# istellartech/GELATO

Measured on AMD Instinct MI355X. Metric: residual+Jacobian evals/sec (and ms/eval), 6-phase x 64-node LGR mesh, higher is better.
Workload: dtype f64

## Files before the change

### gelato_amd/csrc/gel_device.h

```cpp
#pragma once
#include <hip/hip_runtime.h>
#include <stdint.h>

namespace gel {

struct PhaseDev {
  int32_t n, ua, xa;
  int32_t air;
  int32_t air_fd;
  int32_t t_fd;
  int32_t q_fd;
  int32_t engine_on;
  int32_t hold;
  int32_t K;
  int32_t s_vv, s_vq, s_vt, s_qq;
  int32_t doff;
  int32_t toff;
  int64_t voff;
  double thrust, massflow, area, nozzle;
  double mf_um;
};

#ifdef __HIPCC__
template <class T>
__device__ __forceinline__ T load_const(const T* p) {
  return *(const T __attribute__((address_space(4)))*)p;
}
__device__ __forceinline__ int4 load_const_int4(const int4* p) {
  const int32_t* ip = (const int32_t*)p;
  int4 v;
  v.x = load_const(ip); v.y = load_const(ip + 1); v.z = load_const(ip + 2); v.w = load_const(ip + 3);
  return v;
}
__device__ __forceinline__ PhaseDev load_phase(const PhaseDev* g) {
  PhaseDev q;
  q.n = load_const(&g->n); q.ua = load_const(&g->ua); q.xa = load_const(&g->xa);
  q.air = load_const(&g->air); q.air_fd = load_const(&g->air_fd); q.t_fd = load_const(&g->t_fd); q.q_fd = load_const(&g->q_fd); q.engine_on = load_const(&g->engine_on);
  q.hold = load_const(&g->hold); q.K = load_const(&g->K);
  q.s_vv = load_const(&g->s_vv); q.s_vq = load_const(&g->s_vq); q.s_vt = load_const(&g->s_vt); q.s_qq = load_const(&g->s_qq);
  q.doff = load_const(&g->doff); q.toff = load_const(&g->toff); q.voff = load_const(&g->voff);
  q.thrust = load_const(&g->thrust); q.massflow = load_const(&g->massflow); q.area = load_const(&g->area);
  q.nozzle = load_const(&g->nozzle); q.mf_um = load_const(&g->mf_um);
  return q;
}
#endif

// ... 68 lines not shown
```

### gelato_amd/csrc/gel_eval_kernel.h

```cpp
#pragma once

namespace gel {

enum ParkSlot { PK_Q0 = 0, PK_Q1, PK_Q2, PK_Q3, PK_V0, PK_V1, PK_V2, PK_DJJ, PK_LV0, PK_LV1, PK_LV2,
                PK_FP0, PK_FP1, PK_FP2, PK_FP3, PK_FP4, PK_FP5, PK_FP6, PK_FP7, PK_COUNT };
constexpr int kStageLd = 17;
constexpr int kWaveLds = PK_COUNT * 64;
static_assert(kWaveLds >= 64 * kStageLd, "the MFMA staging tile must fit the wave's park region");
constexpr int kCoopStageOff = PK_LV0 * 64;
static_assert(kWaveLds - kCoopStageOff >= 64 * 11, "the cooperative hand-over area must fit behind the early park slots");
constexpr int kXldsPipeFrom = kLongPhaseFrom;
constexpr int kSlabRowsMax = 68, kPackRows = 36, kParkRes = (PK_LV2 + 1) * 64;
constexpr int kPipeSlabK = 8;
constexpr int wave_lds_doubles(bool jac, bool mfma, bool pack, bool split = false, bool longp = true) {
  return jac ? kWaveLds : (!mfma ? kParkRes : (split ? 64 * kStageLd  : (pack ? kParkRes + 4 * 64  : (longp ? 2 * 4 * kPipeSlabK * 11 + 64 * kPipeSlabK  : kSlabRowsMax * 11))));
}
static_assert(wave_lds_doubles(false, true, false, true) >= kParkRes, "residual-only split form: park over the result tile");
static_assert(wave_lds_doubles(false, true, true) >= 64 * 11 && wave_lds_doubles(false, true, false) >= 64 * 11 && wave_lds_doubles(false, true, false, false, false) >= 64 * 11, "hand-over area");
static_assert(wave_lds_doubles(false, true, true) >= kParkRes && wave_lds_doubles(false, true, false) >= kParkRes && wave_lds_doubles(false, true, false, false, false) >= kParkRes, "residual-only park");

constexpr int kSlotPT = 0, kSlotVM = 3, kSlotVP = 6;

#ifndef GEL_MIN_WAVES_PER_SIMD
#define GEL_MIN_WAVES_PER_SIMD 4
#endif
#ifndef GEL_MIN_WAVES_PER_SIMD_PACKJAC
#define GEL_MIN_WAVES_PER_SIMD_PACKJAC 4
#endif
#ifndef GEL_MIN_WAVES_PER_SIMD_RES
#define GEL_MIN_WAVES_PER_SIMD_RES 5
#endif

typedef double gel_double4 __attribute__((ext_vector_type(4)));

#ifndef GEL_CA_CACHE
#define GEL_CA_CACHE 1
#endif
#ifndef GEL_XLDS_A_PF_JAC
#define GEL_XLDS_A_PF_JAC 4
#endif
#ifndef GEL_XLDS_A_PF_RES
#define GEL_XLDS_A_PF_RES 4
#endif
#ifndef GEL_PACK_A_PRELOAD
#define GEL_PACK_A_PRELOAD 1
#endif


// ... 102 lines not shown
  const int dsw = __builtin_amdgcn_readfirstlane(ck.z);
  const int j = PACK ? (lane & 31) : j0 + lane;
  const PhaseDev ph = load_phase((COOP ? f_phases : P.phases) + sec);
  const bool csplit = SPLIT && MFMA && !JAC && B == 1 && res != nullptr && P.split_vel && !((P.unit0 | P.nunits) & 3);
  const bool only_dx = SPLIT && part && (!ph.air || !JAC);
  if (only_dx && !csplit) return;
  const bool lead = !(SPLIT && part);
  const int n = ph.n;
  const bool active = j < n;
  if (!MFMA && !active) return;
  const int jc = active ? j : n - 1;
  const int g = ph.ua + j;
  const int xj = ph.xa + 1 + jc;
  const int M = P.M, N = P.N;

  const double* xb = x + (size_t)b * P.nvars;
  const double* xm = xb;
  const double* xr = xb + M;
  const double* xv = xb + 4 * M;
  const double* xq = xb + 7 * M;
  const double* xu = xb + 11 * M;
  const double* xt = xb + 11 * M + 2 * N;
#define GEL_UNI(v) (PACK ? (v) : wave_uniform(v))
#ifndef GEL_KNOT_VLOAD
#define GEL_KNOT_VLOAD 1
#endif
  int sec_ld = sec;
  if (GEL_KNOT_VLOAD && JAC && !SPLIT) asm volatile("" : "+v"(sec_ld));
  const double to_ld = xt[sec_ld], tf_ld = xt[sec_ld + 1];
  double to = 0.0, tf = 0.0, fds = 0.0, fdt = 0.0;
  const double dx = P.dx, ut = P.ut;
  const double hT = P.hT;
  const double inv_dx = P.inv_dx;
#define GEL_TAKE_KNOT_TIMES()                                   \
  do {                                                          \
    to = GEL_UNI(to_ld); tf = GEL_UNI(tf_ld);                   \
    fds = GEL_UNI(inv_dx * (tf - to) * ut / 2.0);               \
    fdt = GEL_UNI(inv_dx * ut / 2.0);                           \
  } while (0)
  unsigned long long bad = 0;
#define GEL_CHK(v) (bad |= __builtin_amdgcn_ballot_w64(!(fabs(v) <= 1.79769313486231570815e308)))
  const bool packed = SPLIT && P.shard_width != 0;
  const int nn = min(64, n - j0);
  const int sub_hi = packed ? (part ? kSlotVP + 3 * (part - 1) : (ph.air ? 9 : 0)) : 0;
// ... 86 lines not shown
        if (twin_) d_[(W) * (n + lane) + c_] = -(vals_)[c_];                                                           \
      }                                                                                                                \
    }                                                                                                                  \
  } while (0)
#define EMIT_GROUP(W, slot0, vals_, g, k, twin_, okl_)                                                                 \
  do {                                                                                                                 \
    if (coo) {                                                                                                         \
      GEL_COO_EMIT(W, GEL_COO_BASE(g) + (size_t)(W) * n * (k), vals_, okl_, twin_);                                    \
    } else if (okl_) {                                                                                                 \
      _Pragma("unroll") for (int c_ = 0; c_ < (W); c_++) EMIT((slot0) + c_, (vals_)[c_]);                              \
    }                                                                                                                  \
  } while (0)

  constexpr bool XLDS = COOP;
  double me = 0.0, re[3] = {0.0, 0.0, 0.0};
  if (!XLDS) { me = xm[xj]; re[0] = xr[3 * xj]; re[1] = xr[3 * xj + 1]; re[2] = xr[3 * xj + 2]; }
  const double tau = P.tau[ph.toff + jc];
  {
    double q[4] = {0.0, 0.0, 0.0, 0.0}, ve[3] = {0.0, 0.0, 0.0};
    if (!XLDS) {
#pragma unroll
      for (int c = 0; c < 4; c++) q[c] = xq[4 * xj + c];
#pragma unroll
      for (int c = 0; c < 3; c++) ve[c] = xv[3 * xj + c];
    }
    double u0 = 0.0, u1 = 0.0;
    if (!ph.hold) { u0 = xu[2 * (ph.ua + jc)]; u1 = xu[2 * (ph.ua + jc) + 1]; }
    const double djj = JAC ? P.Dt[ph.doff + (size_t)(jc + 1) * n + jc] : 0.0;
    const bool tail1 = MFMA && ((n + 1) & 3) == 1 && n >= 4;
    const int ksteps = tail1 ? (n >> 2) : ((n + 4) >> 2);
    const double* const dcol = P.Dt + ph.doff + (size_t)n * n;
    double dl4[4] = {0, 0, 0, 0};
    if (COOP && tail1) {
      const int rt = PACK ? (wv & 1) : wv;
#pragma unroll
      for (int i = 0; i < 4; i++) dl4[i] = dcol[min(j0 + 16 * rt + (lane >> 4) + 4 * i, n - 1)];
    }
    const double dlast = (SPLIT && tail1) ? dcol[jc] : 0.0;
    double xl[11] = {0, 0, 0, 0, 0, 0, 0, 0, 0, 0, 0};
#define GEL_DX_TAIL_ACC(nct_, xn_of_ct)                                                             \
  do {                                                                                              \
    if (tail1) {                                                                                    \
      _Pragma("unroll") for (int ct = 0; ct < 3; ct++) {                                            \
        if (ct < (nct_)) {                                   \
          const double xn_ = (xn_of_ct);                                                            \
          _Pragma("unroll") for (int i = 0; i < 4; i++) acc[ct][i] = __builtin_fma(dl4[i], xn_, acc[ct][i]); \
        }                                                                                           \
      }                                                                                             \
    }                                                                                               \
  } while (0)

    double m0 = 0.0, q0[4] = {0, 0, 0, 0};
    bool ref0_done = false;
// ... 6 lines not shown
        static_assert(!COOP || kSlabRows * 11 <= kWL, "a slab of state rows must fit the wave's park region");
        lds_double* regions = (lds_double*)lds + park_off;
        const bool h7 = GEL_DX_HOLD7 && !PACK && ph.hold;
        const int ncv = h7 ? 7 : 11;
        const int ncols = ncv * kVecWg;
        const int ct0 = PACK ? (h7 ? 2 : 3) * (wv >> 1) : 0;
        int xoff[3];
#pragma unroll
        for (int ct = 0; ct < 3; ct++) {
          const int c = 16 * (ct0 + ct) + c16;
          const int vb = min(h7 ? c / 7 : c / 11, kVecWg - 1);
          const int col = (c < ncols) ? c - ncv * vb : 0;
          xoff[ct] = PACK ? (vb >> 1) * kWL + (vb & 1) * kPackRows * 11 + col + kq * 11 : vb * kWL + col + kq * 11;
        }
        gel_double4 acc[3];
        const double* ap = P.Dst + (size_t)dsw * 4 + (PACK ? (wv & 1) : wv) * 64 + lane;
        constexpr int kAPF = JAC ? GEL_XLDS_A_PF_JAC : GEL_XLDS_A_PF_RES;
        constexpr int kAllN = PACK ? 9 : kSlabK;
        constexpr bool kAAll = PACK ? (GEL_PACK_A_PRELOAD != 0) : (kAPF >= kSlabK);
        double a_all[kAAll ? kAllN : 1], a_ring[kAAll ? 1 : kAPF];
        if (kAAll) {
#pragma unroll
          for (int ks = 0; ks < kAllN; ks++) a_all[ks] = ap[min(ks, ksteps - 1) * 256];
        } else {
#pragma unroll
          for (int i = 0; i < kAPF; i++) a_ring[i] = ap[min(i, ksteps - 1) * 256];
        }
        constexpr int kRowsStaged = PACK ? 2 * kPackRows : kSlabRows, kExtra = (kRowsStaged - 64) * 11;
        double st[11], sx[(kExtra + 63) / 64];
        {
          const int hv = PACK ? lane / kPackRows : 0;
          const int k = PACK ? lane - kPackRows * hv : lane;
          const double* xs = PACK ? x + (size_t)min(b0 + 2 * wv + hv, B - 1) * P.nvars : xb;
          const int xk = ph.xa + min(k, n);
          st[0] = xs[xk];
#pragma unroll
          for (int c = 0; c < 3; c++) { st[1 + c] = xs[M + 3 * xk + c]; st[4 + c] = xs[4 * M + 3 * xk + c]; }
#pragma unroll
          for (int c = 0; c < 4; c++) st[7 + c] = xs[7 * M + 4 * xk + c];
          constexpr int kER = kRowsStaged - 64, kERs = (kER == 8) ? 3 : 2;
          static_assert(kER == (1 << kERs) && (!PACK || 64 >= kPackRows), "extra rows: a power of two, all in the second half");
#pragma unroll
          for (int i = 0; i < (kExtra + 63) / 64; i++) {
            const int e = min(lane + 64 * i, kExtra - 1);
            const int rr = 64 + (e & (kER - 1)), c = e >> kERs;
            const int kx = min(PACK ? rr - kPackRows : rr, n);
            const double* xe = PACK ? x + (size_t)min(b0 + 2 * wv + 1, B - 1) * P.nvars : xb;
            const int xr_ = ph.xa + kx;
            const int off = (c == 0) ? xr_ : ((c < 4) ? M + 3 * xr_ + (c - 1) : ((c < 7) ? 4 * M + 3 * xr_ + (c - 4) : 7 * M + 4 * xr_ + (c - 7)));
            sx[i] = xe[off];
          }
          lds_double* dst = wave_lds + lane * 11;
#pragma unroll
          for (int c = 0; c < 11; c++) dst[c] = st[c];
#pragma unroll
          for (int i = 0; i < (kExtra + 63) / 64; i++) {
            const int e = min(lane + 64 * i, kExtra - 1);
            wave_lds[(64 + (e & (kER - 1))) * 11 + (e >> kERs)] = sx[i];
          }
        }
        stage_tables_commit(P, lds, tab_mine);
        __syncthreads();
        const int klast = ksteps;
#define GEL_DX_ONE_SLAB(kTiles)                                                                                          \
  do {                                                                                                                   \
// ... 9 lines not shown
            acc[ct] = __builtin_amdgcn_mfma_f64_16x16x4f64(a_all[ks], bl_[ct], ks ? acc[ct] : zero4, 0, 0, 0);           \
        }                                                                                                                \
      }                                                                                                                  \
    } else {                                                                                                             \
       \
      _Pragma("unroll") for (int ct = 0; ct < 3; ct++) acc[ct] = gel_double4{0.0, 0.0, 0.0, 0.0};                        \
      for (int ks = 0; ks < klast; ks += kAPF) {                                                                         \
        _Pragma("unroll") for (int i = 0; i < kAPF; i++) {                                                               \
          if (ks + i < klast) {                                                                        \
            const int ro = (ks + i) * 44;                                                                                \
            double bl_[kTiles];                                                                                          \
            _Pragma("unroll") for (int ct = 0; ct < (kTiles); ct++) bl_[ct] = regions[xoff[ct] + ro];                    \
            _Pragma("unroll") for (int ct = 0; ct < (kTiles); ct++)                                                      \
              acc[ct] = __builtin_amdgcn_mfma_f64_16x16x4f64(a_ring[i], bl_[ct], acc[ct], 0, 0, 0);                      \
          }                                                                                                              \
          a_ring[i] = ap[min(ks + i + kAPF, ksteps - 1) * 256];                                                          \
        }                                                                                                                \
      }                                                                                                                  \
    }                                                                                                                    \
  } while (0)
        if (h7) GEL_DX_ONE_SLAB(2); else GEL_DX_ONE_SLAB(3);
#undef GEL_DX_ONE_SLAB
        GEL_DX_TAIL_ACC(h7 ? 2 : 3, regions[xoff[ct] + (n - kq) * 11]);
        {
          lds_double* src = wave_lds + (half * kPackRows + jc + 1) * 11;
          me = src[0];
#pragma unroll
          for (int c = 0; c < 3; c++) { re[c] = src[1 + c]; ve[c] = src[4 + c]; }
#pragma unroll
          for (int c = 0; c < 4; c++) q[c] = src[7 + c];
          lds_double* src0 = wave_lds + (half * kPackRows) * 11;
          if (!ph.engine_on) m0 = src0[0];
          if (ph.hold) {
#pragma unroll
            for (int c = 0; c < 4; c++) q0[c] = src0[7 + c];
          }
          ref0_done = true;
// ... 43 lines not shown
          xstr[ct] = stride;
        }
        gel_double4 acc[3];
#pragma unroll
        for (int ct = 0; ct < 3; ct++) acc[ct] = gel_double4{0.0, 0.0, 0.0, 0.0};
        typedef const __attribute__((address_space(1))) void* gel_gptr;
        typedef __attribute__((address_space(3))) void* gel_lptr;
        const int xa0 = ph.xa;
        const int s0 = (lane < 16) ? xa0 + 2 * lane : M + 3 * xa0 + 2 * (lane - 16);
        const int s1 = (lane < 48) ? 4 * M + 3 * xa0 + 2 * lane : 7 * M + 4 * xa0 + 2 * (lane - 48);
        const int s2 = 7 * M + 4 * xa0 + 2 * (16 + lane);
        const int a0 = (lane < 16) ? kPipeRows : 3 * kPipeRows, a1 = (lane < 48) ? 3 * kPipeRows : 4 * kPipeRows, a2 = 4 * kPipeRows;
#define GEL_PIPE_ROWS(slab, buf)                                                                                   \
  do {                                                                                                             \
    lds_double* _img = wave_lds + (buf) * kPipeBuf;                                                                \
    __builtin_amdgcn_global_load_lds((gel_gptr)(xb + s0 + (slab) * a0), (gel_lptr)_img, 16, 0, 0);                 \
    __builtin_amdgcn_global_load_lds((gel_gptr)(xb + s1 + (slab) * a1), (gel_lptr)(_img + 128), 16, 0, 0);         \
    if (lane < 48) __builtin_amdgcn_global_load_lds((gel_gptr)(xb + s2 + (slab) * a2), (gel_lptr)(_img + 256), 16, 0, 0); \
  } while (0)
        const double* ap2 = P.Dst + (size_t)dsw * 4 + wv * 64 + (lane & 31) * 2;
        const int khalf = lane >> 5, kmax = ((n + 4) >> 2) - 1;
#define GEL_PIPE_A(pair, k)                                                                                        \
  __builtin_amdgcn_global_load_lds((gel_gptr)(ap2 + (size_t)min((k) + khalf, kmax) * 256), (gel_lptr)(wave_lds + kRingOff + 128 * (pair)), 16, 0, 0)
#define GEL_PIPE_WAIT(N) asm volatile("s_waitcnt vmcnt(%0)" ::"n"(N) : "memory")
        GEL_PIPE_ROWS(0, 0);
#pragma unroll
        for (int pr = 0; pr < kPairs; pr++) GEL_PIPE_A(pr, 2 * pr);
        stage_tables_commit(P, lds, tab_mine);
        GEL_PIPE_WAIT(0);
        __syncthreads();
        const int nslab = (((n + 4) >> 2) + kPipeK - 1) / kPipeK;
        const int own = jc + 1;
        const lds_double* ring = wave_lds + kRingOff + lane;
        for (int sl = 0; sl < nslab; sl++) {
          const int bo = (sl & 1) * kPipeBuf;
          const bool more = sl + 1 < nslab;
          const int k0 = sl * kPipeK;
          if (more) GEL_PIPE_ROWS(sl + 1, (sl + 1) & 1);
// ... 63 lines not shown
          if (c < ncols && (ct < 2 || !h7)) {
#pragma unroll
            for (int i = 0; i < 4; i++) wg_lds[vb * kWL + (16 * wv + kq + 4 * i) * 11 + col] = acc[ct][i];
          }
        }
        __syncthreads();
        if (ghost) return;
        lds_double* row = wave_lds + kHO + lane * 11;
        lm = row[0];
#pragma unroll
        for (int c = 0; c < 3; c++) { lr[c] = row[1 + c]; lv[c] = row[4 + c]; }
#pragma unroll
        for (int c = 0; c < 4; c++) lq[c] = row[7 + c];
      } else if (MFMA && csplit) {
        const int c16 = lane & 15, kq = lane >> 4;
        const double* bp = xm + ph.xa;
        int bs = 1;
        if (c16 >= 1 && c16 < 4) { bp = xr + 3 * ph.xa + (c16 - 1); bs = 3; }
        if (c16 >= 4 && c16 < 7) { bp = xv + 3 * ph.xa + (c16 - 4); bs = 3; }
        if (c16 >= 7) { bp = xq + 4 * ph.xa + ((c16 < 11) ? (c16 - 7) : 0); bs = 4; }
        gel_double4 acc1 = gel_double4{0.0, 0.0, 0.0, 0.0};
        const double* ap1 = P.Dst + (size_t)dsw * 4 + part * 64 + lane;
        const unsigned un = (unsigned)n, ubs = (unsigned)bs;
        if (tail1 && rb) {
          xl[0] = xm[ph.xa + n];
#pragma unroll
          for (int c = 0; c < 3; c++) { xl[1 + c] = xr[3 * (ph.xa + n) + c]; xl[4 + c] = xv[3 * (ph.xa + n) + c]; }
#pragma unroll
          for (int c = 0; c < 4; c++) xl[7 + c] = xq[4 * (ph.xa + n) + c];
        }
        constexpr int kSplitB = SPLITB, kSplitA = 4;
        if (n < kSlabRowsMax) {
          static_assert(!(SPLIT && MFMA && !JAC) || kSlabRowsMax * 11 <= kWL, "the state-row image must fit a wavefront's region");
          lds_double* img = wave_lds + (1 - part) * kWL;
          constexpr int kQRows = kSlabRowsMax / 4, kQ = kQRows * 11;
#pragma unroll
          for (int i = 0; i < (kQ + 63) / 64; i++) {
            const int e = lane + 64 * i;
            const int rl = (e * 373) >> 12, c = e - 11 * rl;
            const int r = kQRows * part + rl;
            if (e < kQ) {
              const int xr_ = ph.xa + min(r, n);
              const int off = (c == 0) ? xr_ : ((c < 4) ? M + 3 * xr_ + (c - 1) : ((c < 7) ? 4 * M + 3 * xr_ + (c - 4) : 7 * M + 4 * xr_ + (c - 7)));
              const double v = xb[off];
              img[r * 11 + c] = (r <= n) ? v : 0.0;
            }
          }
          double a1[kSplitA];
#pragma unroll
          for (int i = 0; i < kSplitA; i++) a1[i] = ap1[min(i, ksteps - 1) * 256];
          __syncthreads();
          const int bo = kq * 11 + ((c16 < 11) ? c16 : 0);
#pragma unroll
          for (int i = 0; i < kSlabRowsMax / 4; i++) {
            if (i < ksteps) {
              acc1 = __builtin_amdgcn_mfma_f64_16x16x4f64(a1[i % kSplitA], img[bo + 44 * i], acc1, 0, 0, 0);
              a1[i % kSplitA] = ap1[min(i + kSplitA, ksteps - 1) * 256];
            }
          }
        } else {
          for (int k0 = 0; k0 < ksteps; k0 += kSplitB) {
            double bl[kSplitB], a1[kSplitA];
#pragma unroll
            for (int i = 0; i < kSplitB; i++) bl[i] = bp[min(4u * (k0 + i) + kq, un) * ubs];
#pragma unroll
            for (int i = 0; i < kSplitA; i++) a1[i] = ap1[min(k0 + i, ksteps - 1) * 256];
#pragma unroll
            for (int i = 0; i < kSplitB; i++) {
              if (k0 + i < ksteps) {
                acc1 = __builtin_amdgcn_mfma_f64_16x16x4f64(a1[i % kSplitA], bl[i], acc1, 0, 0, 0);
                a1[i % kSplitA] = ap1[min(k0 + i + kSplitA, ksteps - 1) * 256];
              }
            }
          }
        }
        lds_double* lead_lds = wave_lds - part * kWL;
#pragma unroll
        for (int i = 0; i < 4; i++) lead_lds[(16 * part + kq + 4 * i) * kStageLd + c16] = acc1[i];
        __syncthreads();
        if (only_dx) return;
        if (rb) {
          lds_double* row = wave_lds + lane * kStageLd;
          lm = row[0];
#pragma unroll
          for (int c = 0; c < 3; c++) { lr[c] = row[1 + c]; lv[c] = row[4 + c]; }
#pragma unroll
          for (int c = 0; c < 4; c++) lq[c] = row[7 + c];
        }
      } else if (MFMA) {
        const int c16 = lane & 15, kq = lane >> 4;
        const double* bp = xm + ph.xa;
        int bs = 1;
        if (c16 >= 1 && c16 < 4) { bp = xr + 3 * ph.xa + (c16 - 1); bs = 3; }
        if (c16 >= 4 && c16 < 7) { bp = xv + 3 * ph.xa + (c16 - 4); bs = 3; }
        if (c16 >= 7) { bp = xq + 4 * ph.xa + ((c16 < 11) ? (c16 - 7) : 0); bs = 4; }
        gel_double4 acc[4];
#pragma unroll
        for (int t = 0; t < 4; t++) acc[t] = gel_double4{0.0, 0.0, 0.0, 0.0};
        const gel_double4* ap = reinterpret_cast<const gel_double4*>(P.Dsw) + (size_t)dsw * 1 + lane;
        const unsigned un = (unsigned)n, ubs = (unsigned)bs;
        if (tail1) {
          xl[0] = xm[ph.xa + n];
#pragma unroll
          for (int c = 0; c < 3; c++) { xl[1 + c] = xr[3 * (ph.xa + n) + c]; xl[4 + c] = xv[3 * (ph.xa + n) + c]; }
#pragma unroll
          for (int c = 0; c < 4; c++) xl[7 + c] = xq[4 * (ph.xa + n) + c];
        }
        constexpr int kSplitB = SPLITB, kSplitA = 2;
        for (int k0 = 0; k0 < ksteps; k0 += kSplitB) {
          double bl[kSplitB];
          gel_double4 a4[kSplitA];
#pragma unroll
          for (int i = 0; i < kSplitB; i++) bl[i] = bp[min(4u * (k0 + i) + kq, un) * ubs];
#pragma unroll
          for (int i = 0; i < kSplitA; i++) a4[i] = ap[min(k0 + i, ksteps - 1) * 64];
#pragma unroll
          for (int i = 0; i < kSplitB; i++) {
            if (k0 + i < ksteps) {
#pragma unroll
              for (int t = 0; t < 4; t++) acc[t] = __builtin_amdgcn_mfma_f64_16x16x4f64(a4[i % kSplitA][t], bl[i], acc[t], 0, 0, 0);
              a4[i % kSplitA] = ap[min(k0 + i + kSplitA, ksteps - 1) * 64];
            }
          }
        }
#pragma unroll
        for (int t = 0; t < 4; t++)
#pragma unroll
          for (int i = 0; i < 4; i++) wave_lds[(16 * t + kq + 4 * i) * kStageLd + c16] = acc[t][i];
        lds_double* row = wave_lds + lane * kStageLd;
        lm = row[0];
#pragma unroll
        for (int c = 0; c < 3; c++) { lr[c] = row[1 + c]; lv[c] = row[4 + c]; }
#pragma unroll
        for (int c = 0; c < 4; c++) lq[c] = row[7 + c];
      } else {
        const double* Dt = P.Dt + ph.doff + j;
        const double* pm = xm + ph.xa;
        const double* pr = xr + 3 * ph.xa;
        const double* pv = xv + 3 * ph.xa;
        const double* pq = xq + 4 * ph.xa;
        for (int i = 0; i <= n; i++) {
          const double d = Dt[(size_t)i * n];
          lm += d * pm[i];
#pragma unroll
          for (int c = 0; c < 3; c++) lr[c] += d * pr[3 * i + c];
#pragma unroll
          for (int c = 0; c < 3; c++) lv[c] += d * pv[3 * i + c];
#pragma unroll
          for (int c = 0; c < 4; c++) lq[c] += d * pq[4 * i + c];
        }
      }
    }
    GEL_TAKE_KNOT_TIMES();
#undef GEL_DX_TAIL_ACC
    if (SPLIT && tail1 && rb) {
      lm = __builtin_fma(dlast, xl[0], lm);
#pragma unroll
      for (int c = 0; c < 3; c++) { lr[c] = __builtin_fma(dlast, xl[1 + c], lr[c]); lv[c] = __builtin_fma(dlast, xl[4 + c], lv[c]); }
#pragma unroll
      for (int c = 0; c < 4; c++) lq[c] = __builtin_fma(dlast, xl[7 + c], lq[c]);
    }
    if (MFMA && !active) return;
    PARK_SET(PK_Q0, q[0]); PARK_SET(PK_Q1, q[1]); PARK_SET(PK_Q2, q[2]); PARK_SET(PK_Q3, q[3]);
    PARK_SET(PK_V0, ve[0]); PARK_SET(PK_V1, ve[1]); PARK_SET(PK_V2, ve[2]);
    if (JAC) PARK_SET(PK_DJJ, djj);
    if (rb) { PARK_SET(PK_LV0, lv[0]); PARK_SET(PK_LV1, lv[1]); PARK_SET(PK_LV2, lv[2]); }
    if (!ref0_done) {
      if (rb && !ph.engine_on) m0 = xm[ph.xa];
      if (rb && ph.hold) {
#pragma unroll
        for (int c = 0; c < 4; c++) q0[c] = xq[4 * ph.xa + c];
      }
    }

    if (JAC && lead) {
      if (coo) {
        const double sc = -(P.kpt * (tf - to));
        double* d_ = P.coo_full + GEL_COO_BASE(CG_PV) + (size_t)3 * j0;
#pragma unroll
        for (int i = 0; i < 3; i++) d_[(cw8 == 512) ? 64 * i + lane : 3 * lane + i] = sc;
      } else if (j == 0) EMIT_AT(packed ? (ph.K - sub_hi) * cw8 : ph.K * n * 8, -(P.kpt * (tf - to)));
      {
        const double pt[3] = {ve[0] * P.kpt, ve[1] * P.kpt, ve[2] * P.kpt};
        EMIT_GROUP(3, kSlotPT, pt, CG_PT, 0, true, true);
      }
    }
// ... 94 lines not shown
                             ((k & 1) ? q_[k ^ 2] : -q_[k ^ 2]) * b_};        \
      EMIT_GROUP(3, ph.s_vq + 3 * k, vq_, CG_VQ, k, false, true);                                                      \
    }                                                                                                                  \
  } while (0)
#define GEL_MASS_CLOSED(tm_)                                                                                           \
  do {                                                                                                                 \
          \
    const double e_ = (fresh_product(me + dx, P.um) - fresh_product(me, P.um)) * inv_m;                                \
    const double k_ = (e_ * (1.0 - e_ * (1.0 - e_))) * (inv_uv * fds);                                                 \
    const double vm_[3] = {(tm_)[0] * k_, (tm_)[1] * k_, (tm_)[2] * k_};                                               \
    EMIT_GROUP(3, kSlotVM, vm_, CG_VM, 0, false, true);                                                                \
  } while (0)
    if (ph.air) {
      EarthHalf eh{1.0, 0.0};
      bool have_eh = false;
#define GEL_NEED_EARTH_ANGLE(ip_, wn_, we_)                                                                            \
  do {                                                                                                                 \
    if (!have_eh && __builtin_amdgcn_ballot_w64(wind_needs_angle(ip_, wn_, we_)) != 0) {                                \
      int jl_ = jc;                                                                                                    \
      if (AERO) asm volatile("" : "+v"(jl_));    \
      const double tau_ = P.tau[ph.toff + jl_];                                                                        \
      const EarthAngle e_ = earth_angle(tau_ * (tf - to) / 2 + (tf + to) / 2);                                         \
      eh.ch = e_.ch; eh.sh = e_.sh; have_eh = true;                                                                    \
    }                                                                                                                  \
  } while (0)
      PosCentreTail pt;
      double cen_rho = 0.0, cen_P = 0.0, cen_inv_a = 0.0;
      double dir2 = 0.0;
      EarthHalf aeh{1.0, 0.0};
      bool have_aeh = false;
#ifndef GEL_AEH
#define GEL_AEH aeh
#endif
#ifndef GEL_X_NOPOS
#define GEL_X_NOPOS 0
#endif
#ifndef GEL_X_NOQUAT
#define GEL_X_NOQUAT 0
#endif
#ifndef GEL_X_NOVEL
#define GEL_X_NOVEL 0
#endif
      const bool aero_on = AERO && akinds != 0;
      const bool a_need_alpha = AERO && (akinds & 5) != 0;
#define GEL_AERO_NEED_EA(ip_, wn_, we_)                                                                                \
  do {                                                                                                                 \
    if (!have_aeh && __builtin_amdgcn_ballot_w64(wind_needs_angle(ip_, wn_, we_)) != 0) {                               \
      int jl_ = jc;                                                                                                    \
      asm volatile("" : "+v"(jl_));    \
      const double tau_ = P.tau[ph.toff + jl_];                                                                        \
      const EarthAngle e_ = earth_angle((tau_ * (tf - to) / 2 + (tf + to) / 2) * P.ut);                                \
      aeh.ch = e_.ch; aeh.sh = e_.sh; have_aeh = true;                                                                 \
    }                                                                                                                  \
  } while (0)
#define GEL_AERO_FETCH()                                                                                               \
  const int ab_[3] = {load_const(&aph->base[0]), load_const(&aph->base[1]), load_const(&aph->base[2])};                \
  const double ax_[3] = {load_const(&aph->ilx[0]), load_const(&aph->ilx[1]), load_const(&aph->ilx[2])};                \
  const int n8_ = 8 * n, j08_ = 8 * j0
#define GEL_AERO_ENTRY(blk, col, a_, nv2_, d_, ind_, rho_, okl_, a_cc, a_ac, a_qc, a_isc, a_ok)                         \
  do {                                                                                                                 \
    double t_ = 0.0, dq_ = 0.0, qp_ = 0.0;                                                                             \
    const double ac_ = a_ac;                                                                                           \
    {                                                                                                                  \
      const double qc_ = a_qc;                                                                                         \
      qp_ = 0.5 * (rho_) * (nv2_);                                                                                     \
// ... 292 lines not shown
              PosPart pd;
              ok = pos_delta(r, k, dlt, pcv, pc, tb, pd);
            }
            asm volatile("" ::: "memory");
            PosPart pq = pos_part(rp, tb, P.barC20);
            double f[3];
            GEL_POS_SWEEP_F(rp, pq, f);
            GEL_POS_SWEEP_EMIT(k, f, !ok);
            if (aero_on && !GEL_X_NOPOS) GEL_AERO_POS(k, rp, pq, !ok);
          }
        }
#undef GEL_AERO_POS
#undef GEL_LOAD_POS_CENTRE
#undef GEL_NEED_EARTH_ANGLE
#undef GEL_AERO_NEED_EA
#undef GEL_AERO_ENTRY
#undef GEL_AERO_FETCH
#undef GEL_POS_SWEEP_F
#undef GEL_POS_SWEEP_EMIT
      }
      if (JAC && lead && ph.t_fd) {
        asm volatile("" ::: "memory");
        const double fcc[3] = {PARK_GET(PK_Q0), PARK_GET(PK_Q1), PARK_GET(PK_Q2)};
        int jl2 = jc;
        if (AERO) asm volatile("" : "+v"(jl2));
        const double tau2 = P.tau[ph.toff + jl2];
        {
          const double r[3] = {fresh_product(re[0], P.up), fresh_product(re[1], P.up), fresh_product(re[2], P.up)};
          const PosPart p2 = pos_part(r, tb, P.barC20);
          const double T2 = ph.thrust - ph.nozzle * p2.P;
          PARK_SET(PK_FP0, p2.shp); PARK_SET(PK_FP1, p2.chp); PARK_SET(PK_FP2, p2.inv_p); PARK_SET(PK_FP3, p2.wn); PARK_SET(PK_FP4, p2.we);
          PARK_SET(PK_FP5, p2.rho); PARK_SET(PK_FP6, p2.inv_a);
          PARK_SET(PK_LV0, p2.g[0]); PARK_SET(PK_LV1, p2.g[1]); PARK_SET(PK_LV2, p2.g[2]);
          PARK_SET(PK_Q0, T2 * PARK_GET(PK_Q3)); PARK_SET(PK_Q1, T2 * PARK_GET(PK_DJJ)); PARK_SET(PK_Q2, T2 * dir2);
        }
#pragma unroll 1
        for (int k = 0; k < 2; k++) {
          asm volatile("" ::: "memory");
          const double to_p = (k == 0) ? to + dx : to;
          const double tf_p = (k == 1) ? tf + dx : tf;
          const double tnp = tau2 * (tf_p - to_p) / 2 + (tf_p + to_p) / 2;
// ... 80 lines not shown
#undef GEL_COO_EMIT
#undef GEL_COO_BASE
#undef EMIT
#undef GEL_CA_BRACKET
#undef GEL_QUAT_CLOSED
#undef GEL_MASS_CLOSED
#undef AEMIT
#undef EMIT_AT
#undef RSTORE
#undef RSTORE_ROWS
#undef RSTORE_LINE
#undef xpose
#undef FDQ
#undef GEL_CHK
#undef GEL_UNI
#undef GEL_TAKE_KNOT_TIMES
#undef PARK_GET
#undef PARK_SET
  if (bad) *(volatile int32_t*)P.flag = 1;
}

__device__ __forceinline__ void signal_done(const ProblemDev& P) {
  if (!P.done_flag) return;
  __threadfence_system();
  __syncthreads();
  if (threadIdx.x == 0) {
    const int old = __hip_atomic_fetch_add(P.done_ctr, 1, __ATOMIC_ACQ_REL, __HIP_MEMORY_SCOPE_AGENT);
    if (old == P.done_total - 1) {
      __hip_atomic_store(P.done_ctr, 0, __ATOMIC_RELAXED, __HIP_MEMORY_SCOPE_AGENT);
      __hip_atomic_store(P.done_flag, P.done_seq, __ATOMIC_RELEASE, __HIP_MEMORY_SCOPE_SYSTEM);
// ... 13 lines not shown
```

### gelato_amd/csrc/gel_tables.h

```cpp
#pragma once
#include <hip/hip_runtime.h>

#include "gel_device.h"
#include "gel_launch.h"
#include "gel_rhs_parts.h"

namespace gel {

#ifndef GEL_BLOCK
#define GEL_BLOCK 256
#endif
constexpr int kBlock = GEL_BLOCK;
static_assert(kAtmDoubles == kAtmTableDoubles, "atmosphere table size mismatch between host and device");

GEL_DEV Tables table_view(const double* base, int Kw, int Kc) {
  Tables tb;
  tb.atm = base;
  tb.wind = base + kAtmDoubles;
  tb.ca = tb.wind + 3 * Kw;
  tb.winds = tb.ca + 2 * Kc;
  tb.cas = tb.winds + 2 * (Kw - 1);
  tb.Kw = Kw;
  tb.Kc = Kc;
  return tb;
}

GEL_DEV double stage_tables_issue(const ProblemDev& P) {
  const int ntab = table_doubles(P.Kw, P.Kc);
  return P.tables[min((int)threadIdx.x, ntab - 1)];
}
GEL_DEV void stage_tables_commit(const ProblemDev& P, double* lds, double mine) {
  const int ntab = table_doubles(P.Kw, P.Kc);
  if ((int)threadIdx.x < ntab) lds[threadIdx.x] = mine;
  for (int i = threadIdx.x + kBlock; i < ntab; i += kBlock) lds[i] = P.tables[i];
}
GEL_DEV Tables stage_tables(const ProblemDev& P, double* lds, bool sync = true) {
  const int ntab = table_doubles(P.Kw, P.Kc);
  for (int i = threadIdx.x; i < ntab; i += blockDim.x) lds[i] = P.tables[i];
  if (sync) __syncthreads();
  return table_view(lds, P.Kw, P.Kc);
}

}
```

Measured before the change: 22.90 million.

## Use scalar-base global and buffer loads with 32-bit lane offsets

Rewrites most global loads in the eval kernel (state vector, tau, differentiation matrices, tables) so the base pointer is made wave-uniform in scalar registers and each lane supplies only a 32-bit byte offset. Several A-operand streams use raw buffer loads with the k-step as a scalar offset. The aim is to cut 64-bit per-lane address arithmetic and VGPR use in the hot MFMA and pointwise paths. The risk is that 32-bit offsets limit addressable size, and the packed-batch base selection adds complexity.

Result: no change. 22.92 million, median of 2 (+0.1%).

```diff
diff --git a/gelato_amd/csrc/gel_device.h b/gelato_amd/csrc/gel_device.h
--- a/gelato_amd/csrc/gel_device.h
+++ b/gelato_amd/csrc/gel_device.h
@@ -30,6 +30,29 @@
   const int32_t* ip = (const int32_t*)p;
   int4 v;
   v.x = load_const(ip); v.y = load_const(ip + 1); v.z = load_const(ip + 2); v.w = load_const(ip + 3);
+  return v;
+}
+typedef const __attribute__((address_space(1))) double* gel_gdp;
+typedef const __attribute__((address_space(1))) char* gel_gchar;
+__device__ __forceinline__ gel_gdp uniform_base(gel_gdp p) {
+  const unsigned long long v = (unsigned long long)p;
+  const unsigned lo = __builtin_amdgcn_readfirstlane((unsigned)v), hi = __builtin_amdgcn_readfirstlane((unsigned)(v >> 32));
+  return (gel_gdp)(((unsigned long long)hi << 32) | lo);
+}
+__device__ __forceinline__ gel_gdp uniform_base(const double* p) { return uniform_base((gel_gdp)p); }
+__device__ __forceinline__ gel_gchar sb_addr(gel_gdp base, unsigned voff, int imm = 0) {
+  return (gel_gchar)base + (unsigned long long)voff + imm;
+}
+__device__ __forceinline__ double load_sb(gel_gdp base, unsigned voff, int imm = 0) { return *(gel_gdp)sb_addr(base, voff, imm); }
+__device__ __forceinline__ double load_sb(const double* base, unsigned voff, int imm = 0) { return load_sb((gel_gdp)base, voff, imm); }
+__device__ __forceinline__ __amdgpu_buffer_rsrc_t load_rsrc(gel_gdp base) {
+  return __builtin_amdgcn_make_buffer_rsrc((void*)base, 0, -1, 0x00020000);
+}
+__device__ __forceinline__ double load_buf(__amdgpu_buffer_rsrc_t rs, unsigned voff, int soff) {
+  typedef unsigned gel_ld_u2 __attribute__((ext_vector_type(2)));
+  const gel_ld_u2 d = __builtin_amdgcn_raw_buffer_load_b64(rs, (int)voff, soff, 0);
+  double v;
+  __builtin_memcpy(&v, &d, 8);
   return v;
 }
 __device__ __forceinline__ PhaseDev load_phase(const PhaseDev* g) {
diff --git a/gelato_amd/csrc/gel_eval_kernel.h b/gelato_amd/csrc/gel_eval_kernel.h
--- a/gelato_amd/csrc/gel_eval_kernel.h
+++ b/gelato_amd/csrc/gel_eval_kernel.h
@@ -32,6 +32,14 @@
 #endif
 
 typedef double gel_double4 __attribute__((ext_vector_type(4)));
+__device__ __forceinline__ gel_double4 load_buf4(__amdgpu_buffer_rsrc_t rs, unsigned voff, int soff) {
+  typedef unsigned gel_ld_u4 __attribute__((ext_vector_type(4)));
+  const gel_ld_u4 lo = __builtin_amdgcn_raw_buffer_load_b128(rs, (int)voff, soff, 0), hi = __builtin_amdgcn_raw_buffer_load_b128(rs, (int)(voff + 16u), soff, 0);
+  gel_double4 v;
+  __builtin_memcpy(&v, &lo, 16);
+  __builtin_memcpy((char*)&v + 16, &hi, 16);
+  return v;
+}
 
 #ifndef GEL_CA_CACHE
 #define GEL_CA_CACHE 1
@@ -164,20 +172,24 @@
   const int xj = ph.xa + 1 + jc;
   const int M = P.M, N = P.N;
 
-  const double* xb = x + (size_t)b * P.nvars;
-  const double* xm = xb;
-  const double* xr = xb + M;
-  const double* xv = xb + 4 * M;
-  const double* xq = xb + 7 * M;
-  const double* xu = xb + 11 * M;
-  const double* xt = xb + 11 * M + 2 * N;
+  const int bu = PACK ? min(b0 + 2 * wv, fB - 1) : b;
+  const gel_gdp xb = uniform_base(x + (size_t)bu * P.nvars);
+  const unsigned nv8 = (unsigned)P.nvars * 8u;
+  const unsigned xh8 = PACK ? (unsigned)(b - bu) * nv8 : 0u;
+#define GEL_XLD(base, idx, c) load_sb((base), (unsigned)(idx) * 8u + xh8, (c) * 8)
+  const gel_gdp xm = xb;
+  const gel_gdp xr = xb + M;
+  const gel_gdp xv = xb + 4 * M;
+  const gel_gdp xq = xb + 7 * M;
+  const gel_gdp xu = xb + 11 * M;
+  const gel_gdp xt = xb + 11 * M + 2 * N;
 #define GEL_UNI(v) (PACK ? (v) : wave_uniform(v))
 #ifndef GEL_KNOT_VLOAD
 #define GEL_KNOT_VLOAD 1
 #endif
   int sec_ld = sec;
   if (GEL_KNOT_VLOAD && JAC && !SPLIT) asm volatile("" : "+v"(sec_ld));
-  const double to_ld = xt[sec_ld], tf_ld = xt[sec_ld + 1];
+  const double to_ld = GEL_XLD(xt, sec_ld, 0), tf_ld = GEL_XLD(xt, sec_ld, 1);
   double to = 0.0, tf = 0.0, fds = 0.0, fdt = 0.0;
   const double dx = P.dx, ut = P.ut;
   const double hT = P.hT;
@@ -294,29 +306,30 @@
 
   constexpr bool XLDS = COOP;
   double me = 0.0, re[3] = {0.0, 0.0, 0.0};
-  if (!XLDS) { me = xm[xj]; re[0] = xr[3 * xj]; re[1] = xr[3 * xj + 1]; re[2] = xr[3 * xj + 2]; }
-  const double tau = P.tau[ph.toff + jc];
+  if (!XLDS) { me = GEL_XLD(xm, xj, 0); re[0] = GEL_XLD(xr, 3 * xj, 0); re[1] = GEL_XLD(xr, 3 * xj, 1); re[2] = GEL_XLD(xr, 3 * xj, 2); }
+  const double tau = load_sb(uniform_base(P.tau + ph.toff), (unsigned)jc * 8u);
   {
     double q[4] = {0.0, 0.0, 0.0, 0.0}, ve[3] = {0.0, 0.0, 0.0};
     if (!XLDS) {
 #pragma unroll
-      for (int c = 0; c < 4; c++) q[c] = xq[4 * xj + c];
-#pragma unroll
-      for (int c = 0; c < 3; c++) ve[c] = xv[3 * xj + c];
+      for (int c = 0; c < 4; c++) q[c] = GEL_XLD(xq, 4 * xj, c);
+#pragma unroll
+      for (int c = 0; c < 3; c++) ve[c] = GEL_XLD(xv, 3 * xj, c);
     }
     double u0 = 0.0, u1 = 0.0;
-    if (!ph.hold) { u0 = xu[2 * (ph.ua + jc)]; u1 = xu[2 * (ph.ua + jc) + 1]; }
-    const double djj = JAC ? P.Dt[ph.doff + (size_t)(jc + 1) * n + jc] : 0.0;
+    if (!ph.hold) { u0 = GEL_XLD(xu, 2 * (ph.ua + jc), 0); u1 = GEL_XLD(xu, 2 * (ph.ua + jc), 1); }
+    const gel_gdp dph = uniform_base(P.Dt + ph.doff);
+    const double djj = JAC ? load_sb(dph, ((unsigned)(jc + 1) * (unsigned)n + (unsigned)jc) * 8u) : 0.0;
     const bool tail1 = MFMA && ((n + 1) & 3) == 1 && n >= 4;
     const int ksteps = tail1 ? (n >> 2) : ((n + 4) >> 2);
-    const double* const dcol = P.Dt + ph.doff + (size_t)n * n;
+    const gel_gdp dcol = dph + (size_t)n * n;
     double dl4[4] = {0, 0, 0, 0};
     if (COOP && tail1) {
       const int rt = PACK ? (wv & 1) : wv;
 #pragma unroll
-      for (int i = 0; i < 4; i++) dl4[i] = dcol[min(j0 + 16 * rt + (lane >> 4) + 4 * i, n - 1)];
+      for (int i = 0; i < 4; i++) dl4[i] = load_sb(dcol, (unsigned)min(j0 + 16 * rt + (lane >> 4) + 4 * i, n - 1) * 8u);
     }
-    const double dlast = (SPLIT && tail1) ? dcol[jc] : 0.0;
+    const double dlast = (SPLIT && tail1) ? load_sb(dcol, (unsigned)jc * 8u) : 0.0;
     double xl[11] = {0, 0, 0, 0, 0, 0, 0, 0, 0, 0, 0};
 #define GEL_DX_TAIL_ACC(nct_, xn_of_ct)                                                             \
   do {                                                                                              \
@@ -353,30 +366,33 @@
           xoff[ct] = PACK ? (vb >> 1) * kWL + (vb & 1) * kPackRows * 11 + col + kq * 11 : vb * kWL + col + kq * 11;
         }
         gel_double4 acc[3];
+        const __amdgpu_buffer_rsrc_t ars_a = load_rsrc(uniform_base(P.Dst + (size_t)dsw * 4 + (PACK ? (wv & 1) : wv) * 64));
+        const unsigned lane8 = (unsigned)lane * 8u;
         const double* ap = P.Dst + (size_t)dsw * 4 + (PACK ? (wv & 1) : wv) * 64 + lane;
+#define GEL_A_AT(k) ((PACK || !JAC) ? load_buf(ars_a, lane8, min((int)(k), ksteps - 1) * 2048) : ap[min((int)(k), ksteps - 1) * 256])
         constexpr int kAPF = JAC ? GEL_XLDS_A_PF_JAC : GEL_XLDS_A_PF_RES;
         constexpr int kAllN = PACK ? 9 : kSlabK;
         constexpr bool kAAll = PACK ? (GEL_PACK_A_PRELOAD != 0) : (kAPF >= kSlabK);
         double a_all[kAAll ? kAllN : 1], a_ring[kAAll ? 1 : kAPF];
         if (kAAll) {
 #pragma unroll
-          for (int ks = 0; ks < kAllN; ks++) a_all[ks] = ap[min(ks, ksteps - 1) * 256];
+          for (int ks = 0; ks < kAllN; ks++) a_all[ks] = GEL_A_AT(ks);
         } else {
 #pragma unroll
-          for (int i = 0; i < kAPF; i++) a_ring[i] = ap[min(i, ksteps - 1) * 256];
+          for (int i = 0; i < kAPF; i++) a_ring[i] = GEL_A_AT(i);
         }
         constexpr int kRowsStaged = PACK ? 2 * kPackRows : kSlabRows, kExtra = (kRowsStaged - 64) * 11;
         double st[11], sx[(kExtra + 63) / 64];
         {
           const int hv = PACK ? lane / kPackRows : 0;
           const int k = PACK ? lane - kPackRows * hv : lane;
-          const double* xs = PACK ? x + (size_t)min(b0 + 2 * wv + hv, B - 1) * P.nvars : xb;
-          const int xk = ph.xa + min(k, n);
-          st[0] = xs[xk];
-#pragma unroll
-          for (int c = 0; c < 3; c++) { st[1 + c] = xs[M + 3 * xk + c]; st[4 + c] = xs[4 * M + 3 * xk + c]; }
-#pragma unroll
-          for (int c = 0; c < 4; c++) st[7 + c] = xs[7 * M + 4 * xk + c];
+          const unsigned xs8 = PACK ? (unsigned)(min(b0 + 2 * wv + hv, B - 1) - bu) * nv8 : 0u;
+          const unsigned xk = (unsigned)(ph.xa + min(k, n));
+          st[0] = load_sb(xm, xk * 8u + xs8);
+#pragma unroll
+          for (int c = 0; c < 3; c++) { st[1 + c] = load_sb(xr, xk * 24u + xs8, 8 * c); st[4 + c] = load_sb(xv, xk * 24u + xs8, 8 * c); }
+#pragma unroll
+          for (int c = 0; c < 4; c++) st[7 + c] = load_sb(xq, xk * 32u + xs8, 8 * c);
           constexpr int kER = kRowsStaged - 64, kERs = (kER == 8) ? 3 : 2;
           static_assert(kER == (1 << kERs) && (!PACK || 64 >= kPackRows), "extra rows: a power of two, all in the second half");
 #pragma unroll
@@ -384,10 +400,10 @@
             const int e = min(lane + 64 * i, kExtra - 1);
             const int rr = 64 + (e & (kER - 1)), c = e >> kERs;
             const int kx = min(PACK ? rr - kPackRows : rr, n);
-            const double* xe = PACK ? x + (size_t)min(b0 + 2 * wv + 1, B - 1) * P.nvars : xb;
+            const gel_gdp xe = PACK ? uniform_base(x + (size_t)min(b0 + 2 * wv + 1, B - 1) * P.nvars) : xb;
             const int xr_ = ph.xa + kx;
             const int off = (c == 0) ? xr_ : ((c < 4) ? M + 3 * xr_ + (c - 1) : ((c < 7) ? 4 * M + 3 * xr_ + (c - 4) : 7 * M + 4 * xr_ + (c - 7)));
-            sx[i] = xe[off];
+            sx[i] = load_sb(xe, (unsigned)off * 8u);
           }
           lds_double* dst = wave_lds + lane * 11;
 #pragma unroll
@@ -427,13 +443,14 @@
             _Pragma("unroll") for (int ct = 0; ct < (kTiles); ct++)                                                      \
               acc[ct] = __builtin_amdgcn_mfma_f64_16x16x4f64(a_ring[i], bl_[ct], acc[ct], 0, 0, 0);                      \
           }                                                                                                              \
-          a_ring[i] = ap[min(ks + i + kAPF, ksteps - 1) * 256];                                                          \
+          a_ring[i] = GEL_A_AT(ks + i + kAPF);                                                                              \
         }                                                                                                                \
       }                                                                                                                  \
     }                                                                                                                    \
   } while (0)
         if (h7) GEL_DX_ONE_SLAB(2); else GEL_DX_ONE_SLAB(3);
 #undef GEL_DX_ONE_SLAB
+#undef GEL_A_AT
         GEL_DX_TAIL_ACC(h7 ? 2 : 3, regions[xoff[ct] + (n - kq) * 11]);
         {
           lds_double* src = wave_lds + (half * kPackRows + jc + 1) * 11;
@@ -507,14 +524,19 @@
 #define GEL_PIPE_ROWS(slab, buf)                                                                                   \
   do {                                                                                                             \
     lds_double* _img = wave_lds + (buf) * kPipeBuf;                                                                \
-    __builtin_amdgcn_global_load_lds((gel_gptr)(xb + s0 + (slab) * a0), (gel_lptr)_img, 16, 0, 0);                 \
-    __builtin_amdgcn_global_load_lds((gel_gptr)(xb + s1 + (slab) * a1), (gel_lptr)(_img + 128), 16, 0, 0);         \
-    if (lane < 48) __builtin_amdgcn_global_load_lds((gel_gptr)(xb + s2 + (slab) * a2), (gel_lptr)(_img + 256), 16, 0, 0); \
-  } while (0)
-        const double* ap2 = P.Dst + (size_t)dsw * 4 + wv * 64 + (lane & 31) * 2;
+    __builtin_amdgcn_global_load_lds((gel_gptr)sb_addr(xb, (unsigned)(s0 + (slab) * a0) * 8u), (gel_lptr)_img, 16, 0, 0);                 \
+    __builtin_amdgcn_global_load_lds((gel_gptr)sb_addr(xb, (unsigned)(s1 + (slab) * a1) * 8u), (gel_lptr)(_img + 128), 16, 0, 0);         \
+    if (lane < 48) __builtin_amdgcn_global_load_lds((gel_gptr)sb_addr(xb, (unsigned)(s2 + (slab) * a2) * 8u), (gel_lptr)(_img + 256), 16, 0, 0); \
+  } while (0)
+        const gel_gdp ap2 = uniform_base(P.Dst + (size_t)dsw * 4 + wv * 64);
+        const unsigned al16 = (unsigned)(lane & 31) * 16u;
         const int khalf = lane >> 5, kmax = ((n + 4) >> 2) - 1;
 #define GEL_PIPE_A(pair, k)                                                                                        \
-  __builtin_amdgcn_global_load_lds((gel_gptr)(ap2 + (size_t)min((k) + khalf, kmax) * 256), (gel_lptr)(wave_lds + kRingOff + 128 * (pair)), 16, 0, 0)
+  do {                                                                                                             \
+    int kk_ = min((int)(k), kmax);                                                                                 \
+    asm volatile("" : "+s"(kk_));                                                                                  \
+    __builtin_amdgcn_global_load_lds((gel_gptr)sb_addr(ap2 + (size_t)kk_ * 256, al16 + (unsigned)min(khalf, kmax - kk_) * 2048u), (gel_lptr)(wave_lds + kRingOff + 128 * (pair)), 16, 0, 0); \
+  } while (0)
 #define GEL_PIPE_WAIT(N) asm volatile("s_waitcnt vmcnt(%0)" ::"n"(N) : "memory")
         GEL_PIPE_ROWS(0, 0);
 #pragma unroll
@@ -608,13 +630,14 @@
         for (int c = 0; c < 4; c++) lq[c] = row[7 + c];
       } else if (MFMA && csplit) {
         const int c16 = lane & 15, kq = lane >> 4;
-        const double* bp = xm + ph.xa;
-        int bs = 1;
-        if (c16 >= 1 && c16 < 4) { bp = xr + 3 * ph.xa + (c16 - 1); bs = 3; }
-        if (c16 >= 4 && c16 < 7) { bp = xv + 3 * ph.xa + (c16 - 4); bs = 3; }
-        if (c16 >= 7) { bp = xq + 4 * ph.xa + ((c16 < 11) ? (c16 - 7) : 0); bs = 4; }
+        int be = ph.xa, bs = 1;
+        if (c16 >= 1 && c16 < 4) { be = M + 3 * ph.xa + (c16 - 1); bs = 3; }
+        if (c16 >= 4 && c16 < 7) { be = 4 * M + 3 * ph.xa + (c16 - 4); bs = 3; }
+        if (c16 >= 7) { be = 7 * M + 4 * ph.xa + ((c16 < 11) ? (c16 - 7) : 0); bs = 4; }
         gel_double4 acc1 = gel_double4{0.0, 0.0, 0.0, 0.0};
-        const double* ap1 = P.Dst + (size_t)dsw * 4 + part * 64 + lane;
+        const __amdgpu_buffer_rsrc_t ars_a1 = load_rsrc(uniform_base(P.Dst + (size_t)dsw * 4 + part * 64));
+        const unsigned lane8 = (unsigned)lane * 8u;
+#define GEL_A1_AT(k) load_buf(ars_a1, lane8, min((int)(k), ksteps - 1) * 2048)
         const unsigned un = (unsigned)n, ubs = (unsigned)bs;
         if (tail1 && rb) {
           xl[0] = xm[ph.xa + n];
@@ -642,32 +665,33 @@
           }
           double a1[kSplitA];
 #pragma unroll
-          for (int i = 0; i < kSplitA; i++) a1[i] = ap1[min(i, ksteps - 1) * 256];
+          for (int i = 0; i < kSplitA; i++) a1[i] = GEL_A1_AT(i);
           __syncthreads();
           const int bo = kq * 11 + ((c16 < 11) ? c16 : 0);
 #pragma unroll
           for (int i = 0; i < kSlabRowsMax / 4; i++) {
             if (i < ksteps) {
               acc1 = __builtin_amdgcn_mfma_f64_16x16x4f64(a1[i % kSplitA], img[bo + 44 * i], acc1, 0, 0, 0);
-              a1[i % kSplitA] = ap1[min(i + kSplitA, ksteps - 1) * 256];
+              a1[i % kSplitA] = GEL_A1_AT(i + kSplitA);
             }
           }
         } else {
           for (int k0 = 0; k0 < ksteps; k0 += kSplitB) {
             double bl[kSplitB], a1[kSplitA];
 #pragma unroll
-            for (int i = 0; i < kSplitB; i++) bl[i] = bp[min(4u * (k0 + i) + kq, un) * ubs];
-#pragma unroll
-            for (int i = 0; i < kSplitA; i++) a1[i] = ap1[min(k0 + i, ksteps - 1) * 256];
+            for (int i = 0; i < kSplitB; i++) bl[i] = load_sb(xb, ((unsigned)be + min(4u * (k0 + i) + kq, un) * ubs) * 8u);
+#pragma unroll
+            for (int i = 0; i < kSplitA; i++) a1[i] = GEL_A1_AT(k0 + i);
 #pragma unroll
             for (int i = 0; i < kSplitB; i++) {
               if (k0 + i < ksteps) {
                 acc1 = __builtin_amdgcn_mfma_f64_16x16x4f64(a1[i % kSplitA], bl[i], acc1, 0, 0, 0);
-                a1[i % kSplitA] = ap1[min(k0 + i + kSplitA, ksteps - 1) * 256];
+                a1[i % kSplitA] = GEL_A1_AT(k0 + i + kSplitA);
               }
             }
           }
         }
+#undef GEL_A1_AT
         lds_double* lead_lds = wave_lds - part * kWL;
 #pragma unroll
         for (int i = 0; i < 4; i++) lead_lds[(16 * part + kq + 4 * i) * kStageLd + c16] = acc1[i];
@@ -683,15 +707,15 @@
         }
       } else if (MFMA) {
         const int c16 = lane & 15, kq = lane >> 4;
-        const double* bp = xm + ph.xa;
-        int bs = 1;
-        if (c16 >= 1 && c16 < 4) { bp = xr + 3 * ph.xa + (c16 - 1); bs = 3; }
-        if (c16 >= 4 && c16 < 7) { bp = xv + 3 * ph.xa + (c16 - 4); bs = 3; }
-        if (c16 >= 7) { bp = xq + 4 * ph.xa + ((c16 < 11) ? (c16 - 7) : 0); bs = 4; }
+        int be = ph.xa, bs = 1;
+        if (c16 >= 1 && c16 < 4) { be = M + 3 * ph.xa + (c16 - 1); bs = 3; }
+        if (c16 >= 4 && c16 < 7) { be = 4 * M + 3 * ph.xa + (c16 - 4); bs = 3; }
+        if (c16 >= 7) { be = 7 * M + 4 * ph.xa + ((c16 < 11) ? (c16 - 7) : 0); bs = 4; }
         gel_double4 acc[4];
 #pragma unroll
         for (int t = 0; t < 4; t++) acc[t] = gel_double4{0.0, 0.0, 0.0, 0.0};
-        const gel_double4* ap = reinterpret_cast<const gel_double4*>(P.Dsw) + (size_t)dsw * 1 + lane;
+        const __amdgpu_buffer_rsrc_t ars_a4 = load_rsrc(uniform_base(P.Dsw + (size_t)dsw * 4));
+        const unsigned lane32 = (unsigned)lane * 32u;
         const unsigned un = (unsigned)n, ubs = (unsigned)bs;
         if (tail1) {
           xl[0] = xm[ph.xa + n];
@@ -705,15 +729,15 @@
           double bl[kSplitB];
           gel_double4 a4[kSplitA];
 #pragma unroll
-          for (int i = 0; i < kSplitB; i++) bl[i] = bp[min(4u * (k0 + i) + kq, un) * ubs];
-#pragma unroll
-          for (int i = 0; i < kSplitA; i++) a4[i] = ap[min(k0 + i, ksteps - 1) * 64];
+          for (int i = 0; i < kSplitB; i++) bl[i] = load_sb(xb, ((unsigned)be + min(4u * (k0 + i) + kq, un) * ubs) * 8u);
+#pragma unroll
+          for (int i = 0; i < kSplitA; i++) a4[i] = load_buf4(ars_a4, lane32, min(k0 + i, ksteps - 1) * 2048);
 #pragma unroll
           for (int i = 0; i < kSplitB; i++) {
             if (k0 + i < ksteps) {
 #pragma unroll
               for (int t = 0; t < 4; t++) acc[t] = __builtin_amdgcn_mfma_f64_16x16x4f64(a4[i % kSplitA][t], bl[i], acc[t], 0, 0, 0);
-              a4[i % kSplitA] = ap[min(k0 + i + kSplitA, ksteps - 1) * 64];
+              a4[i % kSplitA] = load_buf4(ars_a4, lane32, min(k0 + i + kSplitA, ksteps - 1) * 2048);
             }
           }
         }
@@ -728,13 +752,13 @@
 #pragma unroll
         for (int c = 0; c < 4; c++) lq[c] = row[7 + c];
       } else {
-        const double* Dt = P.Dt + ph.doff + j;
-        const double* pm = xm + ph.xa;
-        const double* pr = xr + 3 * ph.xa;
-        const double* pv = xv + 3 * ph.xa;
-        const double* pq = xq + 4 * ph.xa;
+        const __amdgpu_buffer_rsrc_t drs = load_rsrc(dph);
+        const gel_gdp pm = xm + ph.xa;
+        const gel_gdp pr = xr + 3 * ph.xa;
+        const gel_gdp pv = xv + 3 * ph.xa;
+        const gel_gdp pq = xq + 4 * ph.xa;
         for (int i = 0; i <= n; i++) {
-          const double d = Dt[(size_t)i * n];
+          const double d = load_buf(drs, (unsigned)j * 8u, i * n * 8);
           lm += d * pm[i];
 #pragma unroll
           for (int c = 0; c < 3; c++) lr[c] += d * pr[3 * i + c];
@@ -760,10 +784,10 @@
     if (JAC) PARK_SET(PK_DJJ, djj);
     if (rb) { PARK_SET(PK_LV0, lv[0]); PARK_SET(PK_LV1, lv[1]); PARK_SET(PK_LV2, lv[2]); }
     if (!ref0_done) {
-      if (rb && !ph.engine_on) m0 = xm[ph.xa];
+      if (rb && !ph.engine_on) m0 = GEL_XLD(xm, ph.xa, 0);
       if (rb && ph.hold) {
 #pragma unroll
-        for (int c = 0; c < 4; c++) q0[c] = xq[4 * ph.xa + c];
+        for (int c = 0; c < 4; c++) q0[c] = GEL_XLD(xq, 4 * ph.xa, c);
       }
     }
 
@@ -888,12 +912,15 @@
     if (ph.air) {
       EarthHalf eh{1.0, 0.0};
       bool have_eh = false;
+#define GEL_TAU_LATE_BASE uniform_base(P.tau + ph.toff + (PACK ? 0 : j0))
+#define GEL_TAU_LATE_OFF ((unsigned)(PACK ? jc : lane) * 8u)
+#define GEL_TAU_LATE_LD(o) load_buf(load_rsrc(GEL_TAU_LATE_BASE), (o), 0)
 #define GEL_NEED_EARTH_ANGLE(ip_, wn_, we_)                                                                            \
   do {                                                                                                                 \
     if (!have_eh && __builtin_amdgcn_ballot_w64(wind_needs_angle(ip_, wn_, we_)) != 0) {                                \
-      int jl_ = jc;                                                                                                    \
+      unsigned jl_ = GEL_TAU_LATE_OFF;                                                                                 \
       if (AERO) asm volatile("" : "+v"(jl_));    \
-      const double tau_ = P.tau[ph.toff + jl_];                                                                        \
+      const double tau_ = GEL_TAU_LATE_LD(jl_);                                                                        \
       const EarthAngle e_ = earth_angle(tau_ * (tf - to) / 2 + (tf + to) / 2);                                         \
       eh.ch = e_.ch; eh.sh = e_.sh; have_eh = true;                                                                    \
     }                                                                                                                  \
@@ -920,9 +947,9 @@
 #define GEL_AERO_NEED_EA(ip_, wn_, we_)                                                                                \
   do {                                                                                                                 \
     if (!have_aeh && __builtin_amdgcn_ballot_w64(wind_needs_angle(ip_, wn_, we_)) != 0) {                               \
-      int jl_ = jc;                                                                                                    \
+      unsigned jl_ = GEL_TAU_LATE_OFF;                                                                                 \
       asm volatile("" : "+v"(jl_));    \
-      const double tau_ = P.tau[ph.toff + jl_];                                                                        \
+      const double tau_ = GEL_TAU_LATE_LD(jl_);                                                                        \
       const EarthAngle e_ = earth_angle((tau_ * (tf - to) / 2 + (tf + to) / 2) * P.ut);                                \
       aeh.ch = e_.ch; aeh.sh = e_.sh; have_aeh = true;                                                                 \
     }                                                                                                                  \
@@ -1245,6 +1272,9 @@
 #undef GEL_LOAD_POS_CENTRE
 #undef GEL_NEED_EARTH_ANGLE
 #undef GEL_AERO_NEED_EA
+#undef GEL_TAU_LATE_BASE
+#undef GEL_TAU_LATE_OFF
+#undef GEL_TAU_LATE_LD
 #undef GEL_AERO_ENTRY
 #undef GEL_AERO_FETCH
 #undef GEL_POS_SWEEP_F
@@ -1253,9 +1283,9 @@
       if (JAC && lead && ph.t_fd) {
         asm volatile("" ::: "memory");
         const double fcc[3] = {PARK_GET(PK_Q0), PARK_GET(PK_Q1), PARK_GET(PK_Q2)};
-        int jl2 = jc;
+        unsigned jl2 = (unsigned)(PACK ? jc : lane) * 8u;
         if (AERO) asm volatile("" : "+v"(jl2));
-        const double tau2 = P.tau[ph.toff + jl2];
+        const double tau2 = load_buf(load_rsrc(uniform_base(P.tau + ph.toff + (PACK ? 0 : j0))), jl2, 0);
         {
           const double r[3] = {fresh_product(re[0], P.up), fresh_product(re[1], P.up), fresh_product(re[2], P.up)};
           const PosPart p2 = pos_part(r, tb, P.barC20);
@@ -1366,6 +1396,7 @@
 #undef FDQ
 #undef GEL_CHK
 #undef GEL_UNI
+#undef GEL_XLD
 #undef GEL_TAKE_KNOT_TIMES
 #undef PARK_GET
 #undef PARK_SET
diff --git a/gelato_amd/csrc/gel_tables.h b/gelato_amd/csrc/gel_tables.h
--- a/gelato_amd/csrc/gel_tables.h
+++ b/gelato_amd/csrc/gel_tables.h
@@ -27,12 +27,12 @@
 
 GEL_DEV double stage_tables_issue(const ProblemDev& P) {
   const int ntab = table_doubles(P.Kw, P.Kc);
-  return P.tables[min((int)threadIdx.x, ntab - 1)];
+  return load_sb(P.tables, (unsigned)min((int)threadIdx.x, ntab - 1) * 8u);
 }
 GEL_DEV void stage_tables_commit(const ProblemDev& P, double* lds, double mine) {
   const int ntab = table_doubles(P.Kw, P.Kc);
   if ((int)threadIdx.x < ntab) lds[threadIdx.x] = mine;
-  for (int i = threadIdx.x + kBlock; i < ntab; i += kBlock) lds[i] = P.tables[i];
+  for (int i = threadIdx.x + kBlock; i < ntab; i += kBlock) lds[i] = load_buf(load_rsrc((gel_gdp)P.tables), (unsigned)i * 8u, 0);
 }
 GEL_DEV Tables stage_tables(const ProblemDev& P, double* lds, bool sync = true) {
   const int ntab = table_doubles(P.Kw, P.Kc);
```
